# itshawi/data-accelerator

Measured on AMD Instinct MI355X. Metric: events/sec (node) + p99 latency, SimulatedData IoT Flow, higher is better.
Workload: dtype fp64/int64 columns (no reduced precision)

## Files before the change

dxa/io/kafka_device.py:

```python
from __future__ import annotations

import ctypes
from dataclasses import dataclass
from typing import List, Optional, Sequence, Tuple

import numpy as np
import torch

_PLAN_ERRS = {-2: "message format is not v2", -3: "CRC mismatch", -5: "codec decoded on the host only",
              -7: "malformed compressed payload (LZ4 / snappy / zstd)", -8: "dependent-block LZ4 frame", -9: "offset deltas with gaps"}


TORCH_DT = {np.dtype(np.int32): torch.int32, np.dtype(np.int64): torch.int64, np.dtype(np.uint8): torch.uint8}


class Unsupported(Exception):
    """The fetch needs the host decoder."""


_BOUND = False


def _lib():
    global _BOUND
# ... 138 lines not shown
        p, i64, i32 = ctypes.c_void_p, ctypes.c_int64, ctypes.c_int
        L.dxa_kafka_plan_count.argtypes = [p, i64, p, p, p, i32, i32, p, p]
        L.dxa_kafka_plan_fill.argtypes = [p, i64, p, p, p, i32, p] + [p] * 14
        L._plan_many_bound = True
    ns = len(bounds)
    so = np.array([b[0] for b in bounds], np.int64)
    sl = np.array([b[1] - b[0] for b in bounds], np.int64)
    mo = np.array(list(min_offsets), np.int64)
    counts = np.zeros((ns, 4), np.int64)
    nxt = np.zeros(ns, np.int64)
    rc = L.dxa_kafka_plan_count(data.ctypes.data, ns, so.ctypes.data, sl.ctypes.data, mo.ctypes.data,
                                int(verify_crc), threads,
                                counts.ctypes.data, nxt.ctypes.data)
    if rc:
        raise Unsupported(_PLAN_ERRS.get(rc, f"plan error {rc}"))
    nbat, nblk = int(counts[:, 0].sum()), int(counts[:, 1].sum())
    buffer = buffer or PlanBuffer()
    arrs, layout, used = buffer.carve(nbat, nblk)
    rc = L.dxa_kafka_plan_fill(data.ctypes.data, ns, so.ctypes.data, sl.ctypes.data, mo.ctypes.data, threads,
                               counts.ctypes.data, *[arrs[n].ctypes.data for n in
                                                     ("b_count", "b_base", "b_skip", "b_first", "b_nblk", "b_rec0",
                                                      "k_comp_off", "k_comp_len", "k_stored", "k_out_off",
                                                      "k_cap", "b_crc_off", "b_crc_len", "b_crc")])
    if rc:
        raise Unsupported(_PLAN_ERRS.get(rc, f"plan error {rc}"))
    np.subtract(arrs["b_count"], arrs["b_skip"], out=arrs["b_keep"])
    plan = FetchPlan(out_bytes=int(counts[:, 3].sum()), next_offset=int(nxt.max()) if ns else 0,
                     nbytes=int((so + sl).max()) if ns else 0, packed=buffer.buf[:used], layout=layout, **arrs)
    plan.buffer = buffer
    return plan


def merge(plans: Sequence[Tuple[FetchPlan, int]]) -> FetchPlan:
    if not plans:
        return FetchPlan(*(np.zeros(0, t) for t in (np.int32, np.int64, np.int32, np.int32, np.int32, np.int32,
                                                      np.int64, np.int64, np.int32, np.uint8, np.int64, np.int64)),
                         out_bytes=0, next_offset=0)
    cat = lambda k: np.concatenate([getattr(p, k) for p, _ in plans])
    blk0, out0, rec0 = [], [], []
    nb = ob = nr = 0
    for p, _ in plans:
        blk0.append(nb)
        out0.append(ob)
        rec0.append(nr)
        nb += p.nblk
        ob += p.out_bytes
        nr += p.nrec
    return FetchPlan(
        b_count=cat("b_count"), b_base=cat("b_base"), b_skip=cat("b_skip"), b_keep=cat("b_keep"),
        b_first=np.concatenate([p.b_first + b for (p, _), b in zip(plans, blk0)]).astype(np.int32),
        b_nblk=cat("b_nblk"),
        b_rec0=np.concatenate([_rec0(p) + r for (p, _), r in zip(plans, rec0)]),
        k_comp_off=np.concatenate([p.k_comp_off + at for p, at in plans]),
        k_comp_len=cat("k_comp_len"), k_stored=cat("k_stored"),
        k_out_off=np.concatenate([p.k_out_off + o for (p, _), o in zip(plans, out0)]),
        k_cap=cat("k_cap"), out_bytes=ob, next_offset=plans[-1][0].next_offset,
        nbytes=max(at + p.nbytes for p, at in plans),
        b_crc_off=np.concatenate([p.b_crc_off + at for p, at in plans]), b_crc_len=cat("b_crc_len"),
        b_crc=cat("b_crc"))


def _rec0(p: FetchPlan) -> np.ndarray:
    if not p.nbat:
        return np.zeros(0, np.int64)
    c = np.cumsum(p.b_keep, dtype=np.int64)
    return c - p.b_keep


def trim(p: FetchPlan, max_records: int) -> FetchPlan:
    if p.nrec <= max_records:
        return p
    keep = p.b_keep.copy()
    cum = np.cumsum(keep, dtype=np.int64)
    cut = int(np.searchsorted(cum, max_records, side="left"))
    before = int(cum[cut - 1]) if cut else 0
    keep[cut] = max_records - before
    keep[cut + 1:] = 0
    q = FetchPlan(**{**p.__dict__, "b_keep": keep.astype(np.int32)})
    q.b_rec0 = _rec0(q)
    q.next_offset = int(p.b_base[cut] + p.b_skip[cut] + keep[cut])
    return q


class DeviceRecordDecoder:

    def __init__(self, device, chunks: int = 4, copy_stream=None, decode_stream=None, track: bool = True,
                 verify_crc: bool = False):
        self.device = torch.device(device)
        self.verify_crc = verify_crc
        self.crc_stream = torch.cuda.Stream(self.device) if verify_crc else None
        self.chunks = max(1, chunks)
        cus = torch.cuda.get_device_properties(self.device).multi_processor_count
        self.min_blocks_per_chunk = cus * 64
        self.copy_stream = copy_stream or torch.cuda.Stream(self.device)
        self.decode_stream = decode_stream or torch.cuda.Stream(self.device)
        self.track = track
        self.checks: List["DecodeStatus"] = []

    def decode(self, staging: torch.Tensor, plan: FetchPlan):
        from ..engine.processor import RawBatch
        from ..ops import native as N
        dev = self.device
        n = plan.nrec
        if plan.packed is None:
            if not hasattr(self, "_packs"):
                self._packs = PlanBufferPool()
            pb = self._packs.get()
            plan.buffer = pb
            arrs, layout, used = pb.carve(plan.nbat, plan.nblk)
            for name, _dt, _k in _ARRAYS:
                arrs[name][...] = getattr(plan, name)
            packed = pb.buf[:used]
        else:
            packed, layout = plan.packed, plan.layout
        with torch.cuda.stream(self.copy_stream):
            dtab = packed.to(dev, non_blocking=True)
            ddata = torch.empty(plan.nbytes + 32, dtype=torch.uint8, device=dev)
            tab_ev = torch.cuda.Event()
            tab_ev.record(self.copy_stream)
        if getattr(plan, "buffer", None) is not None:
            plan.buffer.release(tab_ev)
        views = {name: dtab[off:off + cnt * np.dtype(dt).itemsize].view(TORCH_DT[np.dtype(dt)])
                 for (name, off, cnt), (_, dt, _k) in zip(layout, _ARRAYS)}
        tabs = [views[k] for k in ("k_comp_off", "k_comp_len", "k_stored", "k_out_off", "k_cap", "b_count",
                                   "b_skip", "b_keep", "b_first", "b_nblk", "b_rec0")]
        crc_tabs = [views[k] for k in ("b_crc_off", "b_crc_len", "b_crc")]
        co, cl, sd, oo, cap, bc, bs, bk, bf, bn, br = tabs
        with torch.cuda.stream(self.decode_stream):
            out = torch.empty(plan.out_bytes + 64, dtype=torch.uint8, device=dev)
            produced = torch.empty(max(1, plan.nblk), dtype=torch.int64, device=dev)
            bstat = torch.empty(max(1, plan.nblk), dtype=torch.int32, device=dev)
            offs = torch.empty(n + 1, dtype=torch.int64, device=dev)
            ends = torch.empty(max(1, n), dtype=torch.int64, device=dev)
            rstat = torch.empty(max(1, plan.nbat), dtype=torch.int32, device=dev)
        self.decode_stream.wait_event(tab_ev)
        st = self.decode_stream.cuda_stream
        nb = plan.nblk
        chunks = max(1, min(self.chunks, nb // max(1, self.min_blocks_per_chunk)))
        kinds = set(np.unique(plan.k_stored[:nb]).tolist()) if nb else set()
        has_gzip, has_snappy, has_zstd = 2 in kinds, 3 in kinds, 4 in kinds
        bounds = np.linspace(0, nb, chunks + 1).astype(np.int64)
        ev_last = tab_ev
        copied = 0
        for k in range(chunks):
            b0, b1 = int(bounds[k]), int(bounds[k + 1])
            if b1 <= b0:
                continue
            lo = copied
            hi = plan.nbytes if b1 == nb else int(plan.k_comp_off[b1])
            copied = hi
            N.call("dxa_memcpy_h2d_async", ddata.data_ptr() + lo, staging.data_ptr() + lo, hi - lo,
                   self.copy_stream.cuda_stream)
            ev = torch.cuda.Event()
            ev.record(self.copy_stream)
            ev_last = ev
            self.decode_stream.wait_event(ev)
            N.call("dxa_lz4_decode_into", N.ptr(ddata), N.ptr(co[b0:b1]), N.ptr(cl[b0:b1]), N.ptr(sd[b0:b1]),
                   N.ptr(oo[b0:b1]), N.ptr(cap[b0:b1]), b1 - b0, N.ptr(out), N.ptr(produced[b0:b1]),
                   N.ptr(bstat[b0:b1]), st)
            for present, entry in ((has_gzip, "dxa_inflate_into"), (has_snappy, "dxa_snappy_decode_into"),
                                   (has_zstd, "dxa_zstd_decode_into")):
                if present:
                    N.call(entry, N.ptr(ddata), N.ptr(co[b0:b1]), N.ptr(cl[b0:b1]), N.ptr(sd[b0:b1]),
                           N.ptr(oo[b0:b1]), N.ptr(cap[b0:b1]), b1 - b0, N.ptr(out), N.ptr(produced[b0:b1]),
                           N.ptr(bstat[b0:b1]), st)
        with torch.cuda.stream(self.decode_stream):
            offs[n:].fill_(plan.out_bytes)
        N.call("dxa_kafka_records", N.ptr(out), plan.nbat, N.ptr(bc), N.ptr(bs), N.ptr(bk), N.ptr(bf), N.ptr(bn),
               N.ptr(br), N.ptr(oo), N.ptr(cap), N.ptr(produced), N.ptr(bstat), N.ptr(offs), N.ptr(ends),
               N.ptr(rstat), st)
        done = torch.cuda.Event()
        done.record(self.decode_stream)
        if self.verify_crc:
            cs = self.crc_stream
            cs.wait_event(ev_last)
            with torch.cuda.stream(cs):
                cstat = torch.empty(max(1, plan.nbat), dtype=torch.int32, device=dev)
            N.call("dxa_kafka_crc", N.ptr(ddata), plan.nbat, *[N.ptr(t) for t in crc_tabs], N.ptr(cstat),
                   cs.cuda_stream)
            cs.wait_event(done)
            with torch.cuda.stream(cs):
                bad = (rstat[:plan.nbat] != 0).sum() + (cstat[:plan.nbat] != 0).sum()
                status = DecodeStatus(bad, cs)
            for t in (ddata, dtab, rstat):
                t.record_stream(cs)
        else:
            with torch.cuda.stream(self.decode_stream):
                status = DecodeStatus((rstat[:plan.nbat] != 0).sum(), self.decode_stream)
        for t in (ddata, produced, bstat, dtab):
            t.record_stream(self.decode_stream)
        if self.track:
            self.checks.append(status)
        self._inflight = [(e, b) for e, b in getattr(self, "_inflight", []) if not e.query()] + \
            [(status.event if self.verify_crc else done, (staging, packed))]
        return RawBatch(out, offs, n, ends=ends[:n], source_bytes=plan.nbytes, status=status), done

    def check(self):
        pending, self.checks = self.checks, []
        bad = sum(s.failed() for s in pending)
        if bad:
            raise DecodeError(f"{bad} Kafka record batch(es) failed to decode on the device")


class DecodeError(ValueError):
    pass


class DecodeStatus:

    __slots__ = ("host", "event")

    def __init__(self, bad: torch.Tensor, stream):
        self.host = torch.empty(1, dtype=torch.int64, pin_memory=True)
        self.host.copy_(bad.reshape(1), non_blocking=True)
        self.event = torch.cuda.Event()
        self.event.record(stream)

    def failed(self) -> int:
        self.event.synchronize()
        return int(self.host[0])

    def raise_if_failed(self, what: str = "batch"):
        bad = self.failed()
        if bad:
            raise DecodeError(f"{what}: {bad} Kafka record batch(es) failed to decode on the device")


_CRC_POLY = 0x82F63B78


def _multmodp(a: int, b: int) -> int:
    p = 0
    m = 1 << 31
    while m:
        if a & m:
            p ^= b
        b = (b >> 1) ^ _CRC_POLY if b & 1 else b >> 1
        m >>= 1
    return p


def _x2n_table():
    t, p = [], 1 << 30
    for _ in range(32):
        t.append(p)
        p = _multmodp(p, p)
    return t


_X2N = _x2n_table()


def _raw_crc(reg: int, data: bytes) -> int:
    for byte in data:
        reg ^= byte
        for _ in range(8):
            reg = (reg >> 1) ^ _CRC_POLY if reg & 1 else reg >> 1
    return reg
# ... 100 lines not shown
```

dxa/ops/csrc/host_kafka.cpp:

```cpp
#include <algorithm>
#include <cstdint>
#include <cstdlib>
#include <cstring>
#include <string>
#include <thread>
#include <vector>
#include <zlib.h>

#include "dxa_lz4.h"
#include "dxa_snappy.h"
#include "dxa_zstd.h"

namespace {

constexpr int64_t kMaxDecoded = (int64_t)1 << 31;

uint32_t g_crc_table[8][256];

bool crc_init() {
  for (uint32_t i = 0; i < 256; ++i) {
    uint32_t c = i;
    for (int k = 0; k < 8; ++k) c = (c & 1) ? (c >> 1) ^ 0x82F63B78u : (c >> 1);
    g_crc_table[0][i] = c;
  }
  for (uint32_t i = 0; i < 256; ++i)
    for (int t = 1; t < 8; ++t) g_crc_table[t][i] = (g_crc_table[t - 1][i] >> 8) ^ g_crc_table[0][g_crc_table[t - 1][i] & 0xff];
  return true;
}

uint32_t crc32c_sw(const uint8_t* p, size_t n, uint32_t c) {
  static const bool init = crc_init();
  (void)init;
  while (n >= 8) {
    uint64_t w;
    std::memcpy(&w, p, 8);
    w ^= c;
    c = g_crc_table[7][w & 0xff] ^ g_crc_table[6][(w >> 8) & 0xff] ^ g_crc_table[5][(w >> 16) & 0xff] ^
        g_crc_table[4][(w >> 24) & 0xff] ^ g_crc_table[3][(w >> 32) & 0xff] ^ g_crc_table[2][(w >> 40) & 0xff] ^
        g_crc_table[1][(w >> 48) & 0xff] ^ g_crc_table[0][w >> 56];
    p += 8;
    n -= 8;
  }
  while (n--) c = (c >> 8) ^ g_crc_table[0][(c ^ *p++) & 0xff];
  return c;
}

#if defined(__x86_64__)
__attribute__((target("sse4.2"))) uint32_t crc32c_hw(const uint8_t* p, size_t n, uint32_t c) {
  uint64_t c64 = c;
  while (n && ((uintptr_t)p & 7)) { c64 = __builtin_ia32_crc32qi((uint32_t)c64, *p++); --n; }
  while (n >= 32) {
    uint64_t w0, w1, w2, w3;
    std::memcpy(&w0, p, 8); std::memcpy(&w1, p + 8, 8); std::memcpy(&w2, p + 16, 8); std::memcpy(&w3, p + 24, 8);
    c64 = __builtin_ia32_crc32di(c64, w0);
    c64 = __builtin_ia32_crc32di(c64, w1);
    c64 = __builtin_ia32_crc32di(c64, w2);
    c64 = __builtin_ia32_crc32di(c64, w3);
    p += 32;
    n -= 32;
  }
  while (n >= 8) { uint64_t w; std::memcpy(&w, p, 8); c64 = __builtin_ia32_crc32di(c64, w); p += 8; n -= 8; }
  while (n--) c64 = __builtin_ia32_crc32qi((uint32_t)c64, *p++);
  return (uint32_t)c64;
}
const bool g_has_sse42 = __builtin_cpu_supports("sse4.2");
#endif

uint32_t crc32c(const uint8_t* p, size_t n) {
#if defined(__x86_64__)
  if (g_has_sse42) return crc32c_hw(p, n, 0xFFFFFFFFu) ^ 0xFFFFFFFFu;
#endif
  return crc32c_sw(p, n, 0xFFFFFFFFu) ^ 0xFFFFFFFFu;
}

inline int64_t be64(const uint8_t* p) {
  uint64_t v = 0;
  for (int i = 0; i < 8; ++i) v = (v << 8) | p[i];
  return (int64_t)v;
}
inline int32_t be32(const uint8_t* p) { return (int32_t)((uint32_t)p[0] << 24 | (uint32_t)p[1] << 16 | (uint32_t)p[2] << 8 | p[3]); }
inline int16_t be16(const uint8_t* p) { return (int16_t)((uint16_t)p[0] << 8 | p[1]); }

inline bool varlong(const uint8_t*& p, const uint8_t* end, int64_t& out) {
  uint64_t v = 0;
  int shift = 0;
  while (p < end) {
    const uint8_t b = *p++;
    v |= (uint64_t)(b & 0x7f) << shift;
    if (!(b & 0x80)) {
      out = (int64_t)(v >> 1) ^ -(int64_t)(v & 1);
      return true;
// ... 502 lines not shown
    if (rc) return rc;
  return 0;
}

__attribute__((visibility("default"))) int dxa_kafka_plan_fill(const uint8_t* data, int64_t nsets,
                                                              const int64_t* set_off, const int64_t* set_len,
                                                              const int64_t* min_off, int threads,
                                                              const int64_t* set_counts, int32_t* b_count,
                                                              int64_t* b_base, int32_t* b_skip, int32_t* b_first,
                                                              int32_t* b_nblk, int64_t* b_rec0, int64_t* k_comp_off,
                                                              int32_t* k_comp_len, uint8_t* k_stored,
                                                              int64_t* k_out_off, int64_t* k_cap, int64_t* b_crc_off,
                                                              int32_t* b_crc_len, int32_t* b_crc) {
  std::vector<int64_t> base((size_t)(4 * (nsets + 1)), 0);
  for (int64_t k = 0; k < nsets; ++k)
    for (int j = 0; j < 4; ++j) base[(size_t)(4 * (k + 1) + j)] = base[(size_t)(4 * k + j)] + set_counts[4 * k + j];
  std::vector<int> rcs((size_t)nsets, 0);
  parallel_sets(nsets, threads, [&](int64_t k) {
    const int64_t b0 = base[(size_t)(4 * k)], k0 = base[(size_t)(4 * k + 1)], r0 = base[(size_t)(4 * k + 2)],
                  o0 = base[(size_t)(4 * k + 3)];
    Plan pl{true, b_count + b0, b_base + b0, b_skip + b0, b_first + b0, b_nblk + b0, b_rec0 + b0,
            k_comp_off + k0, k_comp_len + k0, k_stored + k0, k_out_off + k0, k_cap + k0,
            b_crc_off ? b_crc_off + b0 : nullptr, b_crc_len ? b_crc_len + b0 : nullptr, b_crc ? b_crc + b0 : nullptr};
    int64_t nxt = 0;
    rcs[(size_t)k] = plan_batches(data + set_off[k], set_len[k], min_off[k], pl, &nxt, 0);
    for (int64_t i = 0; i < pl.nbat; ++i) {
      b_first[b0 + i] += (int32_t)k0;
      b_rec0[b0 + i] += r0;
      if (b_crc_off) b_crc_off[b0 + i] += set_off[k];
    }
    for (int64_t i = 0; i < pl.nblk; ++i) {
      k_comp_off[k0 + i] += set_off[k];
      k_out_off[k0 + i] += o0;
    }
  });
  for (int rc : rcs)
    if (rc) return rc;
  return 0;
}

__attribute__((visibility("default"))) uint8_t* dxa_kafka_encode_stream(const uint8_t* vals, const int64_t* offs,
                                                                       int64_t n, int64_t per_batch,
                                                                       int64_t base_offset, int64_t timestamp_ms,
                                                                       int32_t codec, int32_t level,
                                                                       int32_t block_size, int32_t threads,
                                                                       int64_t* out_len) {
  if (per_batch <= 0) return nullptr;
  const int64_t nbat = (n + per_batch - 1) / per_batch;
  std::vector<uint8_t*> parts((size_t)nbat, nullptr);
  std::vector<int64_t> lens((size_t)nbat, 0);
  const int T = threads > 0 ? threads : 1;
  std::vector<std::thread> pool;
  for (int t = 0; t < T; ++t) {
    pool.emplace_back([&, t]() {
      for (int64_t b = t; b < nbat; b += T) {
        const int64_t lo = b * per_batch, hi = lo + per_batch < n ? lo + per_batch : n;
        parts[(size_t)b] = dxa_kafka_encode_lz4(vals, offs + lo, hi - lo, timestamp_ms, codec, level, block_size,
                                                &lens[(size_t)b]);
      }
    });
  }
  for (auto& th : pool) th.join();
  int64_t total = 0;
  bool ok = true;
  for (int64_t b = 0; b < nbat; ++b) {
    ok = ok && parts[(size_t)b] != nullptr;
    total += lens[(size_t)b];
  }
  uint8_t* out = ok ? (uint8_t*)std::malloc((size_t)(total > 0 ? total : 1)) : nullptr;
  int64_t pos = 0;
  for (int64_t b = 0; b < nbat; ++b) {
    if (out) {
      std::memcpy(out + pos, parts[(size_t)b], (size_t)lens[(size_t)b]);
      const int64_t base = base_offset + b * per_batch;
      for (int k = 0; k < 8; ++k) out[pos + k] = (uint8_t)((uint64_t)base >> (56 - 8 * k));
      pos += lens[(size_t)b];
    }
    std::free(parts[(size_t)b]);
  }
  *out_len = total;
  return out;
}
}
```

dxa/ops/csrc/lz4.hip:

```cpp
#include "dxa_common.h"

namespace {

struct InWin {
  const uint8_t* base;
  uintptr_t wb;
  uint4 w;
  __device__ __forceinline__ uint32_t at(int64_t q) {
    const uintptr_t a = reinterpret_cast<uintptr_t>(base + q);
    const uintptr_t b = a & ~(uintptr_t)15;
    if (b != wb) {
      wb = b;
      w = *reinterpret_cast<const uint4*>(b);
    }
    return dxa::window_byte(w, (uint32_t)(a - b));
  }
};

struct OutBuf {
  uint8_t* p;
  int64_t len;
  int head;
  int nacc;
  uint64_t a0, a1;
// ... 286 lines not shown
    int32_t ml = mlc;
    if (ml == 15) {
      uint32_t e;
      do {
        if (ip >= iend) { rc = LZ_TRUNC; break; }
        e = get(ip);
        ++ip;
        ml += (int32_t)e;
      } while (e == 255);
      if (rc != LZ_OK) break;
    }
    ml += 4;
    if (ml > cap - op) { rc = LZ_OVERFLOW; break; }
    const int32_t s0 = op - off;
    if (s0 + (off < ml ? off : ml) > done) {
      __builtin_amdgcn_s_waitcnt(kWaitVm0);
      asm volatile("" ::: "memory");
      done = op;
    }
    if (off >= ml) {
      for (int32_t c = 0; c < ml; c += G)
        if (c + gl < ml) out[op + c + gl] = out[s0 + c + gl];
    } else {
      for (int32_t c = 0; c < ml; c += G) {
        const uint32_t i = (uint32_t)(c + gl);
        if ((int32_t)i < ml) out[op + i] = out[s0 + (int32_t)(i % (uint32_t)off)];
      }
    }
    op += ml;
  }
  if (pml > 0) flush();
  if (rc == LZ_OK && !produced && op != cap) rc = LZ_SIZE;
  if (gl == 0) {
    status[b] = rc;
    if (produced) produced[b] = op;
  }
}

}

DXA_API int dxa_lz4_block_sizes(const void* src, const void* comp_off, const void* comp_len, const void* stored,
                                int64_t nb, int64_t max_block, void* out_len, void* status, void* st) {
  if (nb <= 0) return 0;
  hipLaunchKernelGGL(lz4_sizes_kernel, dim3((unsigned)((nb + 255) / 256)), dim3(256), 0, (hipStream_t)st,
                     (const uint8_t*)src, (const int64_t*)comp_off, (const int32_t*)comp_len, (const uint8_t*)stored,
                     nb, max_block, (int64_t*)out_len, (int32_t*)status);
  return (int)hipGetLastError();
}

template <int G>
static int launch_group(int64_t nb, hipStream_t s, const uint8_t* src, const int64_t* co, const int32_t* cl,
                        const uint8_t* sd, const int64_t* oo, const int64_t* ol, uint8_t* dst, int32_t* status,
                        int64_t* produced) {
  const dim3 grid((unsigned)((nb * G + 255) / 256));
  hipLaunchKernelGGL((lz4_decode_group_kernel<G>), grid, dim3(256), 0, s, src, co, cl, sd, oo, ol, nb, dst, status,
                     produced);
  return (int)hipGetLastError();
}

DXA_API int dxa_lz4_decode(const void* src, const void* comp_off, const void* comp_len, const void* stored,
                           const void* out_off, const void* out_len, int64_t nb, int64_t max_out, void* dst,
                           void* status, void* st) {
  if (nb <= 0) return 0;
  const hipStream_t s = (hipStream_t)st;
  return launch_group<16>(nb, s, (const uint8_t*)src, (const int64_t*)comp_off, (const int32_t*)comp_len,
                          (const uint8_t*)stored, (const int64_t*)out_off, (const int64_t*)out_len, (uint8_t*)dst,
                          (int32_t*)status, (int64_t*)nullptr);
}

DXA_API int dxa_lz4_decode_into(const void* src, const void* comp_off, const void* comp_len, const void* stored,
                                const void* out_off, const void* cap, int64_t nb, void* dst, void* produced,
                                void* status, void* st) {
  if (nb <= 0) return 0;
  const hipStream_t s = (hipStream_t)st;
  const uint8_t* s8 = (const uint8_t*)src;
  const int64_t* co = (const int64_t*)comp_off;
  const int32_t* cl = (const int32_t*)comp_len;
  const uint8_t* sd = (const uint8_t*)stored;
  const int64_t* oo = (const int64_t*)out_off;
  const int64_t* cp = (const int64_t*)cap;
  return launch_group<16>(nb, s, s8, co, cl, sd, oo, cp, (uint8_t*)dst, (int32_t*)status, (int64_t*)produced);
}

DXA_API int dxa_memcpy_h2d_async(void* dst, const void* src, int64_t n, void* st) {
  if (n <= 0) return 0;
  return (int)hipMemcpyAsync(dst, src, (size_t)n, hipMemcpyHostToDevice, (hipStream_t)st);
}
```

dxa/ops/lz4.py:

```python
from __future__ import annotations

import ctypes
import os
from dataclasses import dataclass
from typing import Optional

import numpy as np
import torch

from . import native as N

DEFAULT_BLOCK = 16 * 1024
_HOST = None


class Lz4Error(RuntimeError):
    pass


def _host():
    global _HOST
    if _HOST is None:
        from .serialize import lib
        L = lib()
# ... 106 lines not shown
def frame_table(data) -> FrameTable:
    a = _as_np(data)
    L = _host()
    cs, mb, fe = ctypes.c_int64(0), ctypes.c_int32(0), ctypes.c_int64(0)
    nb = L.dxa_lz4_frame_blocks(a.ctypes.data, a.size, None, None, None, 0, ctypes.byref(cs), ctypes.byref(mb),
                                ctypes.byref(fe))
    if nb == -2:
        raise Lz4Error("dependent-block or dictionary LZ4 frames are decoded on the host only")
    if nb < 0:
        raise Lz4Error("malformed LZ4 frame")
    off = np.zeros(nb, dtype=np.int64)
    ln = np.zeros(nb, dtype=np.int32)
    st = np.zeros(nb, dtype=np.uint8)
    L.dxa_lz4_frame_blocks(a.ctypes.data, a.size, off.ctypes.data, ln.ctypes.data, st.ctypes.data, nb,
                           ctypes.byref(cs), ctypes.byref(mb), ctypes.byref(fe))
    return FrameTable(off, ln, st, cs.value, mb.value, fe.value)


@dataclass
class DeviceFrame:
    data: torch.Tensor
    comp_off: torch.Tensor
    comp_len: torch.Tensor
    stored: torch.Tensor
    out_off: Optional[torch.Tensor]
    out_len: Optional[torch.Tensor]
    content_size: int
    max_block: int
    max_out: int = -1

    @staticmethod
    def from_frame(frame: np.ndarray, block_size: Optional[int] = DEFAULT_BLOCK, pin: bool = False) -> "DeviceFrame":
        t = frame_table(frame)
        padded = np.zeros(frame.size + 32, dtype=np.uint8)
        padded[:frame.size] = frame
        oo = t.out_offsets(block_size)

        def T(x):
            x = torch.from_numpy(np.ascontiguousarray(x))
            return x.pin_memory() if pin else x
        return DeviceFrame(T(padded), T(t.comp_off), T(t.comp_len), T(t.stored),
                           T(oo[0]) if oo else None, T(oo[1]) if oo else None, t.content_size, t.max_block,
                           int(oo[1].max()) if oo and oo[1].size else -1)

    def to(self, device, non_blocking: bool = True) -> "DeviceFrame":
        f = lambda x: None if x is None else x.to(device, non_blocking=non_blocking)
        return DeviceFrame(f(self.data), f(self.comp_off), f(self.comp_len), f(self.stored), f(self.out_off),
                           f(self.out_len), self.content_size, self.max_block, self.max_out)

    def tensors(self):
        return [x for x in (self.data, self.comp_off, self.comp_len, self.stored, self.out_off, self.out_len)
                if x is not None]


def decompress_device(fr: DeviceFrame, check: bool = False) -> torch.Tensor:
    dev = fr.data.device
    if dev.type != "cuda":
        raw = decompress_frame(fr.data.numpy()[:-32])
        out = torch.zeros(len(raw) + 16, dtype=torch.uint8)
        out[:len(raw)] = torch.frombuffer(bytearray(raw), dtype=torch.uint8)
        return out
    nb = int(fr.comp_off.shape[0])
    st = N.stream_handle(dev)
    status = torch.empty(max(nb, 1), dtype=torch.int32, device=dev)
    if fr.out_off is None:
        ln = torch.empty(max(nb, 1), dtype=torch.int64, device=dev)
        N.call("dxa_lz4_block_sizes", N.ptr(fr.data), N.ptr(fr.comp_off), N.ptr(fr.comp_len), N.ptr(fr.stored), nb,
               fr.max_block, N.ptr(ln), N.ptr(status), st)
        ln = ln[:nb]
        off = torch.cumsum(ln, 0) - ln
        total = int(ln.sum().item()) if nb else 0
        max_out = int(ln.max().item()) if nb else 0
        if nb and bool((status[:nb] != 0).any()):
            raise Lz4Error("malformed LZ4 block")
    else:
        off, ln, total, max_out = fr.out_off, fr.out_len, fr.content_size, fr.max_out
    out = torch.empty(total + 16, dtype=torch.uint8, device=dev)
    out[total:].zero_()
    N.call("dxa_lz4_decode", N.ptr(fr.data), N.ptr(fr.comp_off), N.ptr(fr.comp_len), N.ptr(fr.stored), N.ptr(off),
           N.ptr(ln), nb, max_out, N.ptr(out), N.ptr(status), st)
    if check and nb and bool((status[:nb] != 0).any()):
        raise Lz4Error(f"LZ4 block decode failed: status {status[:nb].unique().tolist()}")
    return out


class ChunkedIngest:

    def __init__(self, device, chunks: int = 8, copy_stream=None, decode_stream=None):
        self.device = device
        self.chunks = max(1, chunks)
        self.copy_stream = copy_stream or torch.cuda.Stream(device)
        self.decode_stream = decode_stream or torch.cuda.Stream(device)

    def stage(self, fr: "DeviceFrame"):
        dev = self.device
        if fr.out_off is None:
            raise Lz4Error("chunked ingest needs frames with known block sizes")
        nb = int(fr.comp_off.shape[0])
        total = fr.content_size
        with torch.cuda.stream(self.decode_stream):
            out = torch.empty(total + 16, dtype=torch.uint8, device=dev)
            status = torch.empty(max(nb, 1), dtype=torch.int32, device=dev)
        with torch.cuda.stream(self.copy_stream):
            ddata = torch.empty(fr.data.shape[0], dtype=torch.uint8, device=dev)
        with torch.cuda.stream(self.copy_stream):
            tabs = [x.to(dev, non_blocking=True) for x in (fr.comp_off, fr.comp_len, fr.stored, fr.out_off,
                                                           fr.out_len)]
            tab_ev = torch.cuda.Event()
            tab_ev.record(self.copy_stream)
        comp_off_h = fr.comp_off.numpy() if fr.comp_off.device.type == "cpu" else fr.comp_off.cpu().numpy()
        bounds = np.linspace(0, nb, self.chunks + 1).astype(np.int64)
        nbytes = int(fr.data.shape[0])
        st = self.decode_stream.cuda_stream
        self.decode_stream.wait_event(tab_ev)
        with torch.cuda.stream(self.decode_stream):
            out[total:].zero_()
        for k in range(self.chunks):
            b0, b1 = int(bounds[k]), int(bounds[k + 1])
            if b1 <= b0:
                continue
            lo = 0 if k == 0 else int(comp_off_h[b0])
            hi = nbytes if b1 == nb else int(comp_off_h[b1])
            if fr.data.device.type == "cpu":
                if not fr.data.is_pinned():
                    raise Lz4Error("chunked ingest needs a pinned host frame")
                N.call("dxa_memcpy_h2d_async", ddata.data_ptr() + lo, fr.data.data_ptr() + lo, hi - lo,
                       self.copy_stream.cuda_stream)
            else:
                with torch.cuda.stream(self.copy_stream):
                    ddata[lo:hi].copy_(fr.data[lo:hi], non_blocking=True)
            ev = torch.cuda.Event()
            ev.record(self.copy_stream)
            self.decode_stream.wait_event(ev)
            co, cl, sd, oo, ol = tabs
            N.call("dxa_lz4_decode", N.ptr(ddata), N.ptr(co[b0:b1]), N.ptr(cl[b0:b1]), N.ptr(sd[b0:b1]),
                   N.ptr(oo[b0:b1]), N.ptr(ol[b0:b1]), b1 - b0, fr.max_out, N.ptr(out), N.ptr(status[b0:b1]), st)
        done = torch.cuda.Event()
        done.record(self.decode_stream)
        for t in (ddata, *tabs):
            t.record_stream(self.decode_stream)
        self._inflight = [(e, f) for e, f in getattr(self, "_inflight", []) if not e.query()] + [(done, fr)]
        return out, done
```

dxa/ops/native.py:

```python
from __future__ import annotations

import ctypes
import os
import threading
from pathlib import Path

import torch

_LIB = None
_LOCK = threading.Lock()
_HERE = Path(__file__).resolve().parent
LIB_PATH = Path(os.environ.get("DXA_NATIVE_LIB") or (_HERE / "_native" / "libdxa_kernels.so"))

c_i64 = ctypes.c_int64
c_i32 = ctypes.c_int32
c_p = ctypes.c_void_p

_SIGS = {
    "dxa_byte_map": [c_p, c_p, c_i64, c_p, c_p],
    "dxa_lz4_block_sizes": [c_p, c_p, c_p, c_p, c_i64, c_i64, c_p, c_p, c_p],
    "dxa_lz4_decode": [c_p, c_p, c_p, c_p, c_p, c_p, c_i64, c_i64, c_p, c_p, c_p],
    "dxa_memcpy_h2d_async": [c_p, c_p, c_i64, c_p],
    "dxa_copy_sdma": [c_p, c_p, c_i64],
    "dxa_lz4_decode_into": [c_p, c_p, c_p, c_p, c_p, c_p, c_i64, c_p, c_p, c_p, c_p],
    "dxa_inflate_into": [c_p, c_p, c_p, c_p, c_p, c_p, c_i64, c_p, c_p, c_p, c_p],
    "dxa_snappy_decode_into": [c_p, c_p, c_p, c_p, c_p, c_p, c_i64, c_p, c_p, c_p, c_p],
    "dxa_zstd_decode_into": [c_p, c_p, c_p, c_p, c_p, c_p, c_i64, c_p, c_p, c_p, c_p],
    "dxa_zstd_decode_prof": [c_p, c_p, c_p, c_p, c_p, c_p, c_i64, c_p, c_p, c_p, c_p, c_p],
    "dxa_kafka_records": [c_p, c_i64] + [c_p] * 14,
    "dxa_kafka_crc": [c_p, c_i64, c_p, c_p, c_p, c_p, c_p],
    "dxa_csv_tokenize": [c_p, c_p, c_i64, c_i32, c_i32, c_i32, c_i32, c_p, c_p, c_p, c_p, c_p],
    "dxa_spark_hash_fixed": [c_p, c_i32, c_p, c_i64, c_p, c_p],
    "dxa_spark_hash_str": [c_p, c_p, c_p, c_p, c_i64, c_p, c_p],
    "dxa_serialize_rows": [c_i32, c_p, c_i32, c_i32, c_i32, c_p, c_p, c_p, c_p, c_p],
    "dxa_java_double_dev": [c_p, c_i64, c_p, c_p, c_p],
    "dxa_java_double_hostcheck": [c_p, c_i64, c_p, c_p],
    "dxa_json_parse": [c_p, c_p, c_i64, c_p, c_p, c_i32, c_p, c_p, c_p, c_i32, c_p, c_p, c_p, c_p,
                       c_p, c_p, c_p, c_p, c_p, c_i32, c_p, c_p, c_p, c_p, c_i32, c_i32, c_i32, c_p, c_i32,
                       c_p],
    "dxa_count_newlines": [c_p, c_i64, c_i64, c_p, c_p, c_p],
    "dxa_write_newlines_bits": [c_p, c_i64, c_i64, c_p, c_p, c_i64, c_i64, c_p],
    "dxa_null_counts": [c_p, c_i64, c_i32, c_p, c_p],
    "dxa_hash_i64": [c_p, c_p, c_i64, c_p, ctypes.c_int, c_p],
    "dxa_hash_f64": [c_p, c_p, c_i64, c_p, ctypes.c_int, c_p],
    "dxa_hash_str": [c_p, c_p, c_p, c_p, c_i64, c_p, ctypes.c_int, c_p],
    "dxa_table_insert": [c_p, c_i64, c_p, c_i64, c_p, c_p],
    "dxa_group_ids": [c_p, c_i64, c_p, c_i64, c_p, c_p, c_p, c_p, c_p],
    "dxa_verify_i64": [c_p, c_p, c_p, c_p, c_i64, c_p, c_p],
    "dxa_verify_f64": [c_p, c_p, c_p, c_p, c_i64, c_p, c_p],
    "dxa_verify_str": [c_p, c_p, c_p, c_p, c_p, c_p, c_i64, c_p, c_p],
    "dxa_aggregate": [c_p, c_p, c_p, c_i64, c_i32, c_i32, c_i32, c_p, c_p],
    "dxa_aggregate_multi": [c_p, c_i64, c_i32, c_i32, c_p, c_i32, c_p, c_p, c_p],
    "dxa_aggregate_finish": [c_p, c_i32, c_i32, c_i32, c_p, c_p, c_p, c_p],
    "dxa_partial_finish_size": [],
    "dxa_partial_finish": [c_p, c_p],
    "dxa_group_renumber": [c_p, c_i64, c_p, c_i32, c_p, c_p, c_p],
    "dxa_group_build": [c_p, c_i64, c_p, c_i64, c_p, c_p, c_p, c_p, c_p],
    "dxa_group_build_init": [c_p, c_i64, c_p, c_i64, c_p, c_p, c_p, c_p, c_p],
    "dxa_slot_count": [c_p, c_i64, c_p, c_p],
    "dxa_slot_scatter": [c_p, c_i64, c_p, c_p, c_p, c_p],
    "dxa_probe_count": [c_p, c_p, c_i64, c_p, c_i64, c_p, c_p, c_p, ctypes.c_int, c_p],
    "dxa_probe_write": [c_p, c_i64, c_p, c_p, c_p, c_p, c_p, c_p, ctypes.c_int, c_p],
    "dxa_str_cmp_lit": [c_p, c_p, c_p, c_i64, c_p, c_i32, c_i32, c_p, c_p],
    "dxa_str_eq_col": [c_p, c_p, c_p, c_p, c_p, c_p, c_i64, c_p, c_p],
    "dxa_str_cmp_col": [c_p, c_p, c_p, c_p, c_p, c_p, c_i64, c_i32, c_p, c_p],
    "dxa_str_argext": [c_p, c_i64, c_i32, c_p, c_p, c_p, c_p, c_p, c_i32, c_p, c_p],
    "dxa_str_gather": [c_p, c_p, c_p, c_i64, c_p, c_p, c_p],
    "dxa_str_gather_parts": [c_p, c_i32, c_p],
    "dxa_str_split_count": [c_p, c_p, c_p, c_i64, c_p, c_i32, c_p, c_p],
    "dxa_ts_format": [c_p, c_i64, c_p, c_i32, c_p, c_i32, c_p, c_p],
    "dxa_str_like": [c_p, c_p, c_p, c_i64, c_p, c_i32, c_p, c_p],
    "dxa_str_rlike": [c_p, c_p, c_p, c_i64, c_p, c_i32, c_i32, c_i32, c_p, c_p],
    "dxa_str_regex": [c_p, c_p, c_p, c_i64, c_p, c_i32, c_p, c_i32, c_i32, c_i32, c_p, c_i32, c_p, c_p, c_p, c_p, c_p,
                      c_p, c_p],
    "dxa_gzip_chunks": [c_p, c_i64, c_i32, c_p, c_p, c_i32, c_p, c_p],
    "dxa_gzip_pack": [c_p, c_i32, c_p, c_p, c_i64, c_p, c_p],
    "dxa_str_digest": [c_p, c_p, c_p, c_i64, c_i32, c_p, c_p],
    "dxa_str_crc32": [c_p, c_p, c_p, c_i64, c_p, c_p],
    "dxa_str_encode": [c_p, c_p, c_p, c_i64, c_i32, c_p, c_p, c_p],
    "dxa_f64_str_len": [c_p, c_p, c_i64, c_p, c_p],
    "dxa_f64_str_write": [c_p, c_p, c_i64, c_p, c_p, c_p],
    "dxa_str_to_num": [c_p, c_p, c_p, c_p, c_i64, c_i32, c_p, c_p, c_p],
    "dxa_concat_ws_len": [c_p, c_i32, c_i64, c_i32, c_p, c_p],
    "dxa_concat_ws_write": [c_p, c_i32, c_i64, c_p, c_i32, c_p, c_p, c_p],
    "dxa_str_substr": [c_p, c_p, c_p, c_i64, c_p, c_i64, c_p, c_i64, c_p, c_p, c_p],
    "dxa_str_trim": [c_p, c_p, c_p, c_i64, c_i32, c_p, c_p, c_p],
    "dxa_str_numchars": [c_p, c_p, c_p, c_i64, c_p, c_p],
    "dxa_str_locate": [c_p, c_p, c_p, c_i64, c_p, c_i32, c_i64, c_p, c_p],
    "dxa_str_replace_len": [c_p, c_p, c_p, c_i64, c_p, c_i32, c_i32, c_p, c_p],
    "dxa_str_replace_write": [c_p, c_p, c_p, c_i64, c_p, c_i32, c_p, c_i32, c_p, c_p, c_p],
    "dxa_str_split_write": [c_p, c_p, c_p, c_i64, c_p, c_i32, c_i32, c_p, c_p, c_p],
    "dxa_str_part_size": [],
    "dxa_concat_len": [c_p, c_i32, c_i64, c_p, c_p, c_p],
    "dxa_concat_write": [c_p, c_i32, c_i64, c_p, c_p, c_p, c_p],
    "dxa_concat_part_size": [],
    "dxa_i64_to_str_len": [c_p, c_i64, c_p, c_p],
    "dxa_i64_to_str_write": [c_p, c_i64, c_p, c_p, c_p],
    "dxa_i64_to_str_slots": [c_p, c_i64, c_p, c_p, c_p, c_p],
    "dxa_case_map": [c_p, c_p, c_p, c_i64, c_p, c_p, ctypes.c_int, c_p],
    "dxa_str_to_ts": [c_p, c_p, c_p, c_p, c_i64, c_p, c_p, c_p],
    "dxa_datagen_op_size": [],
    "dxa_datagen_lengths": [c_p, c_i32, c_p, c_i32, c_p, c_i32, ctypes.c_uint64, c_i64, c_i64, c_i64, c_i64, c_p,
                            c_p],
    "dxa_datagen_write": [c_p, c_i32, c_p, c_i32, c_p, c_i32, ctypes.c_uint64, c_i64, c_i64, c_i64, c_i64, c_p,
                          c_p, c_p],
}

_OPTIONAL_SIGS = {}


class NativeError(RuntimeError):
    pass

# ... 101 lines not shown
```

Baseline: 251.6 million.

## Move chunked Kafka ingest loop into native code with batch-aligned occupancy-based cuts

```diff
diff --git a/dxa/io/kafka_device.py b/dxa/io/kafka_device.py
--- a/dxa/io/kafka_device.py
+++ b/dxa/io/kafka_device.py
@@ -244,20 +244,47 @@
     return q
 
 
+def ingest_cuts(b_first, b_nblk, capacity: int, max_launches: int) -> Tuple[np.ndarray, np.ndarray]:
+    L = _lib()
+    p = ctypes.c_void_p
+    L.dxa_ingest_cuts.argtypes = [p, p, ctypes.c_int64, ctypes.c_int64, ctypes.c_int32, p, p]
+    L.dxa_ingest_cuts.restype = ctypes.c_int
+    bf = np.ascontiguousarray(b_first, dtype=np.int32)
+    bn = np.ascontiguousarray(b_nblk, dtype=np.int32)
+    cb = np.zeros(max(1, max_launches) + 1, np.int64)
+    ck = np.zeros(max(1, max_launches) + 1, np.int64)
+    n = L.dxa_ingest_cuts(bf.ctypes.data, bn.ctypes.data, bf.shape[0], capacity, max_launches, cb.ctypes.data,
+                          ck.ctypes.data)
+    if n < 0:
+        raise ValueError("ingest_cuts: batch block tables not back to back, or a non-positive capacity / launch count")
+    return (cb[:n + 1], ck[:n + 1]) if n else (cb[:0], ck[:0])
+
+
 class DeviceRecordDecoder:
 
     def __init__(self, device, chunks: int = 4, copy_stream=None, decode_stream=None, track: bool = True,
-                 verify_crc: bool = False):
+                 verify_crc: bool = False, blocks_per_launch: Optional[int] = None):
         self.device = torch.device(device)
         self.verify_crc = verify_crc
         self.crc_stream = torch.cuda.Stream(self.device) if verify_crc else None
         self.chunks = max(1, chunks)
-        cus = torch.cuda.get_device_properties(self.device).multi_processor_count
-        self.min_blocks_per_chunk = cus * 64
+        if blocks_per_launch is None:
+            from ..ops import lz4
+            blocks_per_launch = lz4.resident_blocks(self.device)
+        self.blocks_per_launch = int(blocks_per_launch)
+        self.launches = 0
         self.copy_stream = copy_stream or torch.cuda.Stream(self.device)
         self.decode_stream = decode_stream or torch.cuda.Stream(self.device)
         self.track = track
         self.checks: List["DecodeStatus"] = []
+
+    @property
+    def min_blocks_per_chunk(self) -> int:
+        return self.blocks_per_launch
+
+    @min_blocks_per_chunk.setter
+    def min_blocks_per_chunk(self, blocks: int):
+        self.blocks_per_launch = int(blocks)
 
     def decode(self, staging: torch.Tensor, plan: FetchPlan):
         from ..engine.processor import RawBatch
@@ -280,14 +307,11 @@
             ddata = torch.empty(plan.nbytes + 32, dtype=torch.uint8, device=dev)
             tab_ev = torch.cuda.Event()
             tab_ev.record(self.copy_stream)
-        if getattr(plan, "buffer", None) is not None:
-            plan.buffer.release(tab_ev)
         views = {name: dtab[off:off + cnt * np.dtype(dt).itemsize].view(TORCH_DT[np.dtype(dt)])
                  for (name, off, cnt), (_, dt, _k) in zip(layout, _ARRAYS)}
         tabs = [views[k] for k in ("k_comp_off", "k_comp_len", "k_stored", "k_out_off", "k_cap", "b_count",
                                    "b_skip", "b_keep", "b_first", "b_nblk", "b_rec0")]
         crc_tabs = [views[k] for k in ("b_crc_off", "b_crc_len", "b_crc")]
-        co, cl, sd, oo, cap, bc, bs, bk, bf, bn, br = tabs
         with torch.cuda.stream(self.decode_stream):
             out = torch.empty(plan.out_bytes + 64, dtype=torch.uint8, device=dev)
             produced = torch.empty(max(1, plan.nblk), dtype=torch.int64, device=dev)
@@ -296,46 +320,26 @@
             ends = torch.empty(max(1, n), dtype=torch.int64, device=dev)
             rstat = torch.empty(max(1, plan.nbat), dtype=torch.int32, device=dev)
         self.decode_stream.wait_event(tab_ev)
-        st = self.decode_stream.cuda_stream
-        nb = plan.nblk
-        chunks = max(1, min(self.chunks, nb // max(1, self.min_blocks_per_chunk)))
-        kinds = set(np.unique(plan.k_stored[:nb]).tolist()) if nb else set()
-        has_gzip, has_snappy, has_zstd = 2 in kinds, 3 in kinds, 4 in kinds
-        bounds = np.linspace(0, nb, chunks + 1).astype(np.int64)
-        ev_last = tab_ev
-        copied = 0
-        for k in range(chunks):
-            b0, b1 = int(bounds[k]), int(bounds[k + 1])
-            if b1 <= b0:
-                continue
-            lo = copied
-            hi = plan.nbytes if b1 == nb else int(plan.k_comp_off[b1])
-            copied = hi
-            N.call("dxa_memcpy_h2d_async", ddata.data_ptr() + lo, staging.data_ptr() + lo, hi - lo,
-                   self.copy_stream.cuda_stream)
-            ev = torch.cuda.Event()
-            ev.record(self.copy_stream)
-            ev_last = ev
-            self.decode_stream.wait_event(ev)
-            N.call("dxa_lz4_decode_into", N.ptr(ddata), N.ptr(co[b0:b1]), N.ptr(cl[b0:b1]), N.ptr(sd[b0:b1]),
-                   N.ptr(oo[b0:b1]), N.ptr(cap[b0:b1]), b1 - b0, N.ptr(out), N.ptr(produced[b0:b1]),
-                   N.ptr(bstat[b0:b1]), st)
-            for present, entry in ((has_gzip, "dxa_inflate_into"), (has_snappy, "dxa_snappy_decode_into"),
-                                   (has_zstd, "dxa_zstd_decode_into")):
-                if present:
-                    N.call(entry, N.ptr(ddata), N.ptr(co[b0:b1]), N.ptr(cl[b0:b1]), N.ptr(sd[b0:b1]),
-                           N.ptr(oo[b0:b1]), N.ptr(cap[b0:b1]), b1 - b0, N.ptr(out), N.ptr(produced[b0:b1]),
-                           N.ptr(bstat[b0:b1]), st)
         with torch.cuda.stream(self.decode_stream):
             offs[n:].fill_(plan.out_bytes)
-        N.call("dxa_kafka_records", N.ptr(out), plan.nbat, N.ptr(bc), N.ptr(bs), N.ptr(bk), N.ptr(bf), N.ptr(bn),
-               N.ptr(br), N.ptr(oo), N.ptr(cap), N.ptr(produced), N.ptr(bstat), N.ptr(offs), N.ptr(ends),
-               N.ptr(rstat), st)
+        hb = [np.ascontiguousarray(getattr(plan, k), dtype=dt)
+              for k, dt in (("b_first", np.int32), ("b_nblk", np.int32), ("k_comp_off", np.int64),
+                            ("k_stored", np.uint8))]
+        launches = ctypes.c_int32(0)
+        with torch.cuda.device(dev):
+            N.call("dxa_kafka_ingest", staging.data_ptr(), N.ptr(ddata), plan.nbytes, hb[0].ctypes.data,
+                   hb[1].ctypes.data, plan.nbat, hb[2].ctypes.data, hb[3].ctypes.data, plan.nblk,
+                   *[N.ptr(t) for t in tabs], N.ptr(out), N.ptr(produced), N.ptr(bstat), N.ptr(offs), N.ptr(ends),
+                   N.ptr(rstat), self.blocks_per_launch or 0, self.chunks, self.copy_stream.cuda_stream,
+                   self.decode_stream.cuda_stream, ctypes.byref(launches))
+        self.launches = launches.value
+        if getattr(plan, "buffer", None) is not None:
+            plan.buffer.release(tab_ev)
         done = torch.cuda.Event()
         done.record(self.decode_stream)
         if self.verify_crc:
             cs = self.crc_stream
-            cs.wait_event(ev_last)
+            cs.wait_stream(self.copy_stream)
             with torch.cuda.stream(cs):
                 cstat = torch.empty(max(1, plan.nbat), dtype=torch.int32, device=dev)
             N.call("dxa_kafka_crc", N.ptr(ddata), plan.nbat, *[N.ptr(t) for t in crc_tabs], N.ptr(cstat),
diff --git a/dxa/ops/csrc/dxa_ingest_cuts.h b/dxa/ops/csrc/dxa_ingest_cuts.h
--- /dev/null
+++ b/dxa/ops/csrc/dxa_ingest_cuts.h
@@ -0,0 +1,57 @@
+#pragma once
+#include <algorithm>
+#include <cstdint>
+#include <vector>
+
+namespace dxa {
+
+inline int ingest_cuts(const int32_t* b_first, const int32_t* b_nblk, int64_t nbat, int64_t capacity,
+                       int max_launches, int64_t* cut_batch, int64_t* cut_block) {
+  if (capacity <= 0 || max_launches <= 0 || nbat < 0) return -1;
+  int64_t nblk = 0;
+  for (int64_t i = 0; i < nbat; ++i) {
+    if (b_first[i] != nblk || b_nblk[i] < 0) return -1;
+    nblk += b_nblk[i];
+  }
+  if (nblk == 0) return 0;
+  std::vector<int64_t> pos, bat;
+  for (int64_t i = 1; i < nbat; ++i)
+    if (b_first[i] > 0 && b_first[i] < nblk && (pos.empty() || pos.back() != b_first[i])) {
+      pos.push_back(b_first[i]);
+      bat.push_back(i);
+    }
+  const int64_t D = (int64_t)pos.size();
+  int64_t want = std::min<int64_t>(max_launches, (nblk + capacity - 1) / capacity);
+  want = std::min(want, D + 1);
+  std::vector<int64_t> cuts;
+  int64_t prev = -1;
+  for (int64_t k = 1; k < want; ++k) {
+    const int64_t target = (k * nblk + want - 1) / want;
+    int64_t j = std::lower_bound(pos.begin(), pos.end(), target) - pos.begin();
+    if (j == D || (j > 0 && target - pos[j - 1] <= pos[j] - target)) --j;
+    j = std::min(std::max(j, prev + 1), D - want + k);
+    cuts.push_back(j);
+    prev = j;
+  }
+  for (int64_t i = 0; i < nbat; ++i) {
+    if (b_nblk[i] <= capacity) continue;
+    for (const int64_t edge : {(int64_t)b_first[i], (int64_t)b_first[i] + b_nblk[i]}) {
+      if (edge <= 0 || edge >= nblk || (int64_t)cuts.size() + 1 >= max_launches) continue;
+      const int64_t j = std::lower_bound(pos.begin(), pos.end(), edge) - pos.begin();
+      const auto at = std::lower_bound(cuts.begin(), cuts.end(), j);
+      if (at == cuts.end() || *at != j) cuts.insert(at, j);
+    }
+  }
+  const int L = (int)cuts.size() + 1;
+  cut_batch[0] = 0;
+  cut_block[0] = 0;
+  for (int k = 1; k < L; ++k) {
+    cut_batch[k] = bat[(size_t)cuts[(size_t)k - 1]];
+    cut_block[k] = pos[(size_t)cuts[(size_t)k - 1]];
+  }
+  cut_batch[L] = nbat;
+  cut_block[L] = nblk;
+  return L;
+}
+
+}
diff --git a/dxa/ops/csrc/host_kafka.cpp b/dxa/ops/csrc/host_kafka.cpp
--- a/dxa/ops/csrc/host_kafka.cpp
+++ b/dxa/ops/csrc/host_kafka.cpp
@@ -7,6 +7,7 @@
 #include <vector>
 #include <zlib.h>
 
+#include "dxa_ingest_cuts.h"
 #include "dxa_lz4.h"
 #include "dxa_snappy.h"
 #include "dxa_zstd.h"
@@ -675,3 +676,10 @@
   return out;
 }
 }
+
+extern "C" __attribute__((visibility("default"))) int dxa_ingest_cuts(const int32_t* b_first, const int32_t* b_nblk,
+                                                                     int64_t nbat, int64_t capacity,
+                                                                     int32_t max_launches, int64_t* cut_batch,
+                                                                     int64_t* cut_block) {
+  return dxa::ingest_cuts(b_first, b_nblk, nbat, capacity, max_launches, cut_batch, cut_block);
+}
diff --git a/dxa/ops/csrc/kafka_ingest.hip b/dxa/ops/csrc/kafka_ingest.hip
--- /dev/null
+++ b/dxa/ops/csrc/kafka_ingest.hip
@@ -0,0 +1,131 @@
+#include <hip/hip_runtime.h>
+
+#include <mutex>
+
+#include "dxa_common.h"
+#include "dxa_ingest_cuts.h"
+
+DXA_API int64_t dxa_lz4_resident_blocks(int device);
+DXA_API int dxa_lz4_decode_into(const void* src, const void* comp_off, const void* comp_len, const void* stored,
+                                const void* out_off, const void* cap, int64_t nb, void* dst, void* produced,
+                                void* status, void* st);
+DXA_API int dxa_inflate_into(const void* src, const void* comp_off, const void* comp_len, const void* kind,
+                             const void* out_off, const void* cap, int64_t nb, void* dst, void* produced, void* status,
+                             void* st);
+DXA_API int dxa_snappy_decode_into(const void* src, const void* comp_off, const void* comp_len, const void* kind,
+                                   const void* out_off, const void* cap, int64_t nb, void* dst, void* produced,
+                                   void* status, void* st);
+DXA_API int dxa_zstd_decode_into(const void* src, const void* comp_off, const void* comp_len, const void* kind,
+                                 const void* out_off, const void* cap, int64_t nb, void* dst, void* produced,
+                                 void* status, void* st);
+DXA_API int dxa_kafka_records(const uint8_t* buf, int64_t nbat, const int32_t* b_count, const int32_t* b_skip,
+                              const int32_t* b_keep, const int32_t* b_first, const int32_t* b_nblk,
+                              const int64_t* b_rec0, const int64_t* k_out_off, const int64_t* k_cap,
+                              const int64_t* produced, const int32_t* blk_status, int64_t* starts, int64_t* ends,
+                              int32_t* bstatus, void* stream);
+
+namespace {
+
+constexpr int kMaxLaunches = 64;
+constexpr int kMaxDevices = 64;
+constexpr int kPoolEvents = 32;
+
+struct EventPool {
+  std::mutex mu;
+  hipEvent_t ev[kMaxDevices][kPoolEvents] = {};
+  int next[kMaxDevices] = {};
+  int64_t capacity[kMaxDevices] = {};
+
+  hipError_t get(int dev, hipEvent_t* out) {
+    std::lock_guard<std::mutex> g(mu);
+    hipEvent_t& e = ev[dev][next[dev]];
+    next[dev] = (next[dev] + 1) % kPoolEvents;
+    if (!e) {
+      const hipError_t rc = hipEventCreateWithFlags(&e, hipEventDisableTiming);
+      if (rc != hipSuccess) {
+        e = nullptr;
+        return rc;
+      }
+    }
+    *out = e;
+    return hipSuccess;
+  }
+};
+
+EventPool g_pool;
+
+#define DXA_TRY(expr)                     \
+  do {                                    \
+    const int rc_ = (int)(expr);          \
+    if (rc_ != 0) return rc_;             \
+  } while (0)
+
+}
+
+DXA_API int dxa_kafka_ingest(const uint8_t* staging, uint8_t* ddata, int64_t nbytes, const int32_t* h_b_first,
+                             const int32_t* h_b_nblk, int64_t nbat, const int64_t* h_comp_off, const uint8_t* h_kind,
+                             int64_t nblk, const int64_t* co, const int32_t* cl, const uint8_t* sd, const int64_t* oo,
+                             const int64_t* cap, const int32_t* bc, const int32_t* bs, const int32_t* bk,
+                             const int32_t* bf, const int32_t* bn, const int64_t* br, uint8_t* out,
+                             int64_t* produced, int32_t* bstat, int64_t* starts, int64_t* ends, int32_t* rstat,
+                             int64_t capacity, int32_t max_launches, void* copy_stream, void* decode_stream,
+                             int32_t* launches) {
+  const hipStream_t cs = (hipStream_t)copy_stream, ds = (hipStream_t)decode_stream;
+  if (launches) *launches = 0;
+  if (nbat <= 0 && nbytes <= 0) return 0;
+  int dev = 0;
+  DXA_TRY(hipGetDevice(&dev));
+  if (dev < 0 || dev >= kMaxDevices) return (int)hipErrorInvalidDevice;
+  if (capacity <= 0) {
+    {
+      std::lock_guard<std::mutex> g(g_pool.mu);
+      capacity = g_pool.capacity[dev];
+    }
+    if (capacity <= 0) {
+      capacity = dxa_lz4_resident_blocks(dev);
+      if (capacity <= 0) return capacity < 0 ? (int)-capacity : (int)hipErrorInvalidValue;
+      std::lock_guard<std::mutex> g(g_pool.mu);
+      g_pool.capacity[dev] = capacity;
+    }
+  }
+  int64_t cut_batch[kMaxLaunches + 1], cut_block[kMaxLaunches + 1];
+  const int maxl = max_launches < 1 ? 1 : (max_launches > kMaxLaunches ? kMaxLaunches : max_launches);
+  int L = dxa::ingest_cuts(h_b_first, h_b_nblk, nbat, capacity, maxl, cut_batch, cut_block);
+  if (L < 0 || (L > 0 && cut_block[L] != nblk)) return -1;
+  if (launches) *launches = L;
+  if (L == 0) {
+    if (nblk != 0) return -1;
+    L = 1;
+    cut_block[0] = cut_block[1] = 0;
+  }
+  int64_t copied = 0;
+  for (int k = 0; k < L; ++k) {
+    const int64_t b0 = cut_block[k], b1 = cut_block[k + 1];
+    const int64_t hi = k + 1 == L ? nbytes : h_comp_off[b1];
+    if (hi < copied || hi > nbytes) return -1;
+    if (hi > copied)
+      DXA_TRY(hipMemcpyAsync(ddata + copied, staging + copied, (size_t)(hi - copied), hipMemcpyHostToDevice, cs));
+    copied = hi;
+    hipEvent_t ev = nullptr;
+    DXA_TRY(g_pool.get(dev, &ev));
+    DXA_TRY(hipEventRecord(ev, cs));
+    DXA_TRY(hipStreamWaitEvent(ds, ev, 0));
+    const int64_t nb = b1 - b0;
+    DXA_TRY(dxa_lz4_decode_into(ddata, co + b0, cl + b0, sd + b0, oo + b0, cap + b0, nb, out, produced + b0,
+                                bstat + b0, ds));
+    bool has[5] = {false, false, false, false, false};
+    for (int64_t b = b0; b < b1; ++b)
+      if (h_kind[b] < 5) has[h_kind[b]] = true;
+    if (has[2])
+      DXA_TRY(dxa_inflate_into(ddata, co + b0, cl + b0, sd + b0, oo + b0, cap + b0, nb, out, produced + b0,
+                               bstat + b0, ds));
+    if (has[3])
+      DXA_TRY(dxa_snappy_decode_into(ddata, co + b0, cl + b0, sd + b0, oo + b0, cap + b0, nb, out, produced + b0,
+                                     bstat + b0, ds));
+    if (has[4])
+      DXA_TRY(dxa_zstd_decode_into(ddata, co + b0, cl + b0, sd + b0, oo + b0, cap + b0, nb, out, produced + b0,
+                                   bstat + b0, ds));
+  }
+  DXA_TRY(dxa_kafka_records(out, nbat, bc, bs, bk, bf, bn, br, oo, cap, produced, bstat, starts, ends, rstat, ds));
+  return 0;
+}
diff --git a/dxa/ops/csrc/lz4.hip b/dxa/ops/csrc/lz4.hip
--- a/dxa/ops/csrc/lz4.hip
+++ b/dxa/ops/csrc/lz4.hip
@@ -392,6 +392,21 @@
   return launch_group<16>(nb, s, s8, co, cl, sd, oo, cp, (uint8_t*)dst, (int32_t*)status, (int64_t*)produced);
 }
 
+DXA_API int64_t dxa_lz4_resident_blocks(int device) {
+  hipError_t e = hipSuccess;
+  if (device < 0 && (e = hipGetDevice(&device)) != hipSuccess) return -(int64_t)e;
+  int cus = 0, wgs = 0, cur = 0;
+  if ((e = hipDeviceGetAttribute(&cus, hipDeviceAttributeMultiprocessorCount, device)) != hipSuccess)
+    return -(int64_t)e;
+  if ((e = hipGetDevice(&cur)) != hipSuccess) return -(int64_t)e;
+  if (cur != device && (e = hipSetDevice(device)) != hipSuccess) return -(int64_t)e;
+  e = hipOccupancyMaxActiveBlocksPerMultiprocessor(&wgs, lz4_decode_group_kernel<16>, 256, 0);
+  if (cur != device) (void)hipSetDevice(cur);
+  if (e != hipSuccess) return -(int64_t)e;
+  if (cus <= 0 || wgs <= 0) return -(int64_t)hipErrorInvalidValue;
+  return (int64_t)cus * wgs * (256 / 16);
+}
+
 DXA_API int dxa_memcpy_h2d_async(void* dst, const void* src, int64_t n, void* st) {
   if (n <= 0) return 0;
   return (int)hipMemcpyAsync(dst, src, (size_t)n, hipMemcpyHostToDevice, (hipStream_t)st);
diff --git a/dxa/ops/lz4.py b/dxa/ops/lz4.py
--- a/dxa/ops/lz4.py
+++ b/dxa/ops/lz4.py
@@ -212,6 +212,16 @@
     if check and nb and bool((status[:nb] != 0).any()):
         raise Lz4Error(f"LZ4 block decode failed: status {status[:nb].unique().tolist()}")
     return out
+
+
+def resident_blocks(device=None) -> int:
+    fn = N.lib().dxa_lz4_resident_blocks
+    fn.argtypes, fn.restype = [ctypes.c_int], ctypes.c_int64
+    idx = -1 if device is None else torch.device(device).index
+    n = int(fn(-1 if idx is None else idx))
+    if n <= 0:
+        raise N.NativeError(f"dxa_lz4_resident_blocks failed with HIP error {-n}")
+    return n
 
 
 class ChunkedIngest:
diff --git a/dxa/ops/native.py b/dxa/ops/native.py
--- a/dxa/ops/native.py
+++ b/dxa/ops/native.py
@@ -29,6 +29,8 @@
     "dxa_zstd_decode_prof": [c_p, c_p, c_p, c_p, c_p, c_p, c_i64, c_p, c_p, c_p, c_p, c_p],
     "dxa_kafka_records": [c_p, c_i64] + [c_p] * 14,
     "dxa_kafka_crc": [c_p, c_i64, c_p, c_p, c_p, c_p, c_p],
+    "dxa_kafka_ingest": [c_p, c_p, c_i64, c_p, c_p, c_i64, c_p, c_p, c_i64] + [c_p] * 17 +
+                        [c_i64, c_i32, c_p, c_p, c_p],
     "dxa_csv_tokenize": [c_p, c_p, c_i64, c_i32, c_i32, c_i32, c_i32, c_p, c_p, c_p, c_p, c_p],
     "dxa_spark_hash_fixed": [c_p, c_i32, c_p, c_i64, c_p, c_p],
     "dxa_spark_hash_str": [c_p, c_p, c_p, c_p, c_i64, c_p, c_p],
```

Result: no change. 250.9 million (-0.3%).
